# ZechengLi19/CIM

Hardware: AMD Instinct MI355X
Metric: images/sec training step (ResNet-50 VOC, ~1k proposals/img) at 1/2/4/8 GPU (higher is better)
Workload: dtype fp32

## Files before the change

### cim_amd/_lib.py

```python
import ctypes
import os

from ctypes import c_float, c_int, c_longlong, c_void_p

HERE = os.path.dirname(os.path.abspath(__file__))
LIB_PATH = os.environ.get("CIM_HIP_LIB") or os.path.join(HERE, "libcim_hip.so")

_P = c_void_p
SIGNATURES = {
    "cim_roi_align_fwd": [_P, _P, _P] + [c_int] * 6 + [c_float, c_int, c_int, _P],
    "cim_roi_align_fwd_ws": [_P, _P, _P] + [c_int] * 6 + [c_float, c_int, c_int, _P, _P],
    "cim_roi_align_maskcat_fwd_ws": [_P, _P, _P, _P] + [c_int] * 6 + [c_float, c_int, c_int, _P, _P],
    "cim_roi_align_wino7_pair_fwd": [_P, _P, _P, _P, _P] + [c_int] * 7 + [c_float, c_int, c_int, _P, _P],
    "cim_roi_align_bwd_ws": [_P, _P, _P] + [c_int] * 6 + [c_float, c_int, c_int, _P, c_int, _P, _P],
    "cim_roi_align_maskcat_bwd_ws": [_P, _P, _P, _P] + [c_int] * 6 + [c_float, c_int, c_int, _P, c_int, _P, _P],
    "cim_roi_align_bwd_workspace": [c_int, c_int, c_int, c_int],
    "cim_roi_align_bwd_scratch": [c_int, c_int, c_int, c_int, c_int],
    "cim_roi_align_bwd": [_P, _P, _P] + [c_int] * 6 + [c_float, c_int, c_int, _P, _P],
    "cim_roi_align_maskcat_fwd": [_P, _P, _P, _P] + [c_int] * 6 + [c_float, c_int, c_int, _P],
    "cim_roi_align_maskcat_bwd": [_P, _P, _P, _P] + [c_int] * 6 + [c_float, c_int, c_int, _P, _P],
    "cim_roi_align_forms": [c_int] * 9 + [_P] * 3,
    "cim_maxpool2d_out_size": [c_int, c_int, c_int, c_int],
    "cim_maxpool2d_fwd": [_P, _P, _P, c_int, c_int, c_int, c_int, c_int, c_int, _P],
    "cim_maxpool2d_bwd": [_P, _P, _P, c_int, c_int, c_int, c_int, c_int, c_int, _P],
    "cim_upsample_nearest_fwd": [_P, _P, c_int, c_int, c_int, c_int, c_int, _P],
    "cim_upsample_nearest_bwd": [_P, _P, c_int, c_int, c_int, c_int, _P],
    "cim_image_prep": [_P, c_int, c_int, _P, c_int, c_int, c_longlong, c_int, ctypes.c_double, c_int, _P, _P],
    "cim_mask_pack": [_P, _P, c_int, c_int, _P],
    "cim_mask_iou_pair": [_P, c_int, c_int, _P, _P, _P, _P],
    "cim_asy_flag": [_P, c_int, c_float, _P, _P],
    "cim_asy_prep": [_P, c_int, _P, c_int, _P, _P, _P],
    "cim_mining_step": [_P, _P, _P],
    "cim_mining_lds_bytes": [c_int, c_int],
    "cim_mining_sync_bytes": [],
    "cim_gemm_small_splits": [c_int, c_int, c_int],
    "cim_gemm_small_f32": [_P, _P, _P] + [c_int] * 8 + [_P, _P, _P, _P, _P, c_float, _P, c_int, c_int, _P, _P],
    "cim_conv1x1_bwd_workspace": [c_int, c_int, c_int, c_int],
    "cim_conv1x1_bn_act_bwd": [_P] * 8 + [c_float, c_int] + [_P] * 5 + [c_int] * 4 + [_P, _P, _P, _P, _P, c_int] + [c_int, _P, _P, c_float] + [_P] * 4 + [c_int],
    "cim_bn_part_finish": [_P, c_int, _P],
    "cim_conv3x3_nchw_splits": [c_int] * 5,
    "cim_conv3x3_nchw_f32": [_P, _P, _P] + [c_int] * 6 + [_P, _P, _P, _P, _P, c_float, _P, c_int, c_int, _P, _P],
    "cim_conv7x7_nchw_f32": [_P, _P, _P] + [c_int] * 5 + [_P, _P, _P, _P, c_float, c_int, _P],
    "cim_conv3x3_nchw_bwd_workspace": [c_int] * 6,
    "cim_conv3x3_dx_parts": [c_int] * 3,
    "cim_conv3x3_nchw_bn_act_bwd": [_P] * 8 + [c_float, c_int] + [_P] * 5 + [c_int] * 7 + [_P, _P, _P, _P, _P, c_int] + [c_int, _P, _P, c_float] + [_P] * 4,
    "cim_conv3x3_wt_multi": [_P, c_int, _P],
    "cim_bn_act_fwd": [_P, _P, _P, _P, _P, _P, c_float, _P, c_int, c_int, c_int, c_int, _P],
    "cim_bn_act_bwd_chunks": [c_int, c_int, c_int],
    "cim_bn_act_bwd": [_P, _P, _P, _P, _P, _P, c_float, _P, _P, _P, _P, c_int, c_int, c_int, c_int, _P],
    "cim_sgd_multi": [_P, _P, c_int, c_float, c_int, _P],
    "cim_adam_multi": [_P, _P, c_int, ctypes.c_double, ctypes.c_double, ctypes.c_double, c_int, _P],
    "cim_gemm_pair_splits": [c_int, c_int, c_int],
    "cim_gemm_pair": [_P, _P, _P, _P] + [c_int] * 6 + [c_int, c_int, c_int, c_int, _P, _P, _P, _P, c_int, c_int, c_int, _P],
    "cim_gemm_pair_batched": [_P, _P, _P] + [c_int] * 6 + [c_int, c_int, c_int, c_longlong, c_longlong, c_longlong,
                              _P, _P, c_int, c_int, c_int, _P],
    "cim_pair_scales": [_P, c_int, _P, _P, c_int, c_int, _P],
    "cim_pair_split": [_P, _P, c_int, c_int, c_int, c_int, c_int, c_int, c_longlong, c_longlong, _P, _P, _P],
    "cim_pair_amax": [_P, c_longlong, _P, _P],
    "cim_pair_masked_stats": [_P, _P, c_int, c_int, _P, _P, _P],
    "cim_wino7_flatten_bwd_dy_pair": [_P, _P, _P, _P, _P, _P, _P, c_int, c_int, c_int, _P],
    "cim_wino7_pair_scales": [_P, c_int, _P, c_int, _P, _P],
    "cim_wino7_input_pair": [_P, _P, _P, c_int, c_int, c_int, _P],
    "cim_wino7_filter_pair": [_P, _P, _P, c_int, c_int, _P],
    "cim_wino7_dy_pair": [_P, _P, _P, c_int, c_int, c_int, c_int, _P],
    "cim_wino7_output_amax": [_P, _P, _P, c_int, c_int, c_int, _P, _P],
    "cim_flatten_chw_pair": [_P, _P, _P, c_int, c_int, c_int, c_int, _P],
    "cim_flatten_chw_bwd_bias": [_P, _P, _P, _P, c_int, c_int, c_int, _P],
    "cim_wino_dx_adjoint_output": [_P, _P, c_int, c_int, c_int, c_int, _P],
    "cim_wino7_dx_maskfold": [_P, _P, _P, c_int, c_int, _P],
    "cim_wino_wgrad_output": [_P, _P, c_int, c_int, c_int, _P],
    "cim_losses_fwd": [_P, _P],
    "cim_linear_bias_f32": [_P, _P, _P, _P, c_int, c_int, c_int, c_int, _P, _P],
    "cim_loss_finish": [_P, c_int, _P, _P],
    "cim_loss_grad_combine": [_P] * 8 + [c_int, c_int, c_int, _P],
    "cim_head_act_fwd": [_P, _P, _P, c_int, c_int, c_int, _P],
    "cim_head_act_bwd": [_P, _P, _P, _P, c_int, c_int, c_int, _P],
    "cim_detect_ws_bytes": [c_int, c_int],
    "cim_detect_nms_limit": [_P, c_int, _P, c_int, c_int, c_float, c_float, c_int, _P, _P, _P, _P, _P],
    "cim_detect_corloc": [_P, c_int, c_int, c_int, _P, _P],
    "cim_batch_detect_ws_bytes": [_P, c_int, c_int],
    "cim_batch_detect_nms_limit": [_P, c_int, _P, _P, _P, c_int, c_int, c_float, c_float, c_int, _P, _P, _P, _P, _P, _P, _P],
    "cim_segm_words": [c_int, c_int],
    "cim_segm_pack": [_P, _P, c_longlong, c_int, c_int, c_int, _P, _P],
    "cim_segm_area": [_P, c_int, c_int, _P, _P],
    "cim_segm_rle_count": [_P, c_int, c_int, c_int, _P, _P],
    "cim_segm_rle_write": [_P, c_int, c_int, c_int, _P, _P, _P, _P],
    "cim_segm_rle_decode_ws_bytes": [c_longlong],
    "cim_segm_rle_decode": [_P, _P, _P, c_int, c_int, c_int, _P, _P, _P],
    "cim_segm_image_ws_bytes": [c_int, c_int, c_longlong],
    "cim_segm_record_bytes": [c_int, c_int, c_int, c_int],
    "cim_segm_eval_image": [_P, c_int, _P, c_int, c_int, _P, _P, c_int, c_int, c_int, c_longlong, _P, _P, _P, c_int, _P, c_int,
                            _P, _P, _P],
    "cim_segm_accumulate_ws_bytes": [c_longlong, c_int, c_int, c_int],
    "cim_segm_accumulate": [_P, c_int, c_longlong, c_int, _P, _P, _P, c_int, _P, c_int, _P, c_int, c_int, c_int, _P, _P, _P, _P,
                            _P],
# ... 80 lines not shown
```

### cim_amd/csrc/conv1x1.hip

```cpp
#include "common.h"
#include "../../include/cim_hip.h"

#ifndef CIM_BODY_PRIO_LEVEL
#define CIM_BODY_PRIO_LEVEL 3
#endif
#if CIM_BODY_PRIO_LEVEL > 0
#define CIM_BODY_PRIO() __builtin_amdgcn_s_setprio(CIM_BODY_PRIO_LEVEL)
#else
#define CIM_BODY_PRIO()
#endif
namespace {

#ifndef CIM_SMALL_BK
#define CIM_SMALL_BK 32
#endif
#ifndef CIM_SMALL_ABL
#define CIM_SMALL_ABL 0
#endif
constexpr int SBM = 64, SBN = 64, SBK = CIM_SMALL_BK;
constexpr int SLD = 68;
typedef float f32x16 __attribute__((ext_vector_type(16)));
typedef float f32x4u __attribute__((ext_vector_type(4), aligned(4)));
__device__ __forceinline__ float4 ld4(const float* p) {
    const f32x4u v = *reinterpret_cast<const f32x4u*>(p);
// ... 11 lines not shown
    const float* mask; const float* mgamma; const float* mvar; float meps;
    const float* mxr; const float* mmean; float* mpart; int mparts;
    int res_w, res_ws, res_hw;
};
struct InputBn { const float* y; const float* gamma; const float* var; float eps;
                 const float* xr; const float* mean; float* part; };

typedef unsigned int u32x4 __attribute__((ext_vector_type(4)));
typedef __amdgpu_buffer_rsrc_t rsrc_t;
__device__ __forceinline__ rsrc_t make_rsrc(const float* p, long long floats) {
    return __builtin_amdgcn_make_buffer_rsrc(const_cast<float*>(p), 0, (int)(unsigned)(floats * 4), 0x00020000);
}
__device__ __forceinline__ float4 bld4(rsrc_t r, unsigned byte_off) {
    const u32x4 v = __builtin_amdgcn_raw_buffer_load_b128(r, byte_off, 0, 0);
    return make_float4(__uint_as_float(v.x), __uint_as_float(v.y), __uint_as_float(v.z), __uint_as_float(v.w));
}
__device__ __forceinline__ float bld1(rsrc_t r, unsigned byte_off) {
    return __uint_as_float(__builtin_amdgcn_raw_buffer_load_b32(r, byte_off, 0, 0));
}
constexpr unsigned OOB = 0x7fffffffu;
__host__ __device__ __forceinline__ long long tile_extent(bool RC, int rows, int K, int ld) {
    return RC ? (long long)(K - 1) * ld + rows : (long long)(rows - 1) * ld + K;
}
template <bool RC, int ROWS>
__device__ __forceinline__ unsigned tile_off(int ld, int r0, int k0, int p) {
    int r, k;
    if (RC) { k = k0 + p / (ROWS / 4); r = r0 + (p % (ROWS / 4)) * 4; return ((unsigned)k * ld + r) * 4u; }
    r = r0 + p % ROWS; k = k0 + (p / ROWS) * 4;
    return ((unsigned)r * ld + k) * 4u;
}
template <bool RC, int ROWS>
__device__ __forceinline__ float4 tile_ktail(float4 v, int K, int k0, int p) {
    if (!RC) {
        const int left = K - (k0 + (p / ROWS) * 4);
        v.x = left > 0 ? v.x : 0.0f; v.y = left > 1 ? v.y : 0.0f; v.z = left > 2 ? v.z : 0.0f; v.w = left > 3 ? v.w : 0.0f;
    }
    return v;
}

template <bool RC, int ROWS>
__device__ __forceinline__ void tile_store(float* __restrict__ S, float4 v, int p) {
    if (RC) {
        const int k = p / (ROWS / 4), r = (p % (ROWS / 4)) * 4;
        *reinterpret_cast<float4*>(S + k * SLD + r) = v;
    } else {
        const int r = p % ROWS, k = (p / ROWS) * 4;
        S[(k + 0) * SLD + r] = v.x;
        S[(k + 1) * SLD + r] = v.y;
        S[(k + 2) * SLD + r] = v.z;
        S[(k + 3) * SLD + r] = v.w;
    }
}

__device__ __forceinline__ float small_value(const SmallArgs& g, int row, int col, float v, float& s1, float& s2) {
    const size_t o = (size_t)row * g.ldc + col;
    float y = v;
    if (g.bn) {
        const float a = g.gamma[row] * rsqrtf(g.var[row] + g.eps);
        y = fmaf(v, a, g.beta[row] - g.mean[row] * a);
    }
    if (g.res) {
        if (g.res_w == 0) y += g.res[o];
        else {
            const int py = col / g.res_w, px = col - py * g.res_w;
            if (!((py | px) & 1)) y += g.res[(size_t)row * g.res_hw + (py >> 1) * g.res_ws + (px >> 1)];
        }
    }
    if (g.colbias) y += g.colbias[col];
    if (g.relu) y = fmaxf(y, 0.0f);
    if (g.mask) {
        const bool on = g.mask[o] > 0.0f;
        if (g.mpart && on) { s1 += y; s2 = fmaf(y, g.mxr[o] - g.mmean[row], s2); }
        y = on ? y * (g.mgamma[row] * rsqrtf(g.mvar[row] + g.meps)) : 0.0f;
    }
    return y;
}
__device__ __forceinline__ void small_finish(const SmallArgs& g, int row, int col, float v, float& s1, float& s2) {
    const size_t o = (size_t)row * g.ldc + col;
    if (g.Xraw) g.Xraw[o] = v;
    g.C[o] = small_value(g, row, col, v, s1, s2);
}
__device__ __forceinline__ void small_finish(const SmallArgs& g, int row, int col, float v) {
    float s1 = 0.0f, s2 = 0.0f;
    small_finish(g, row, col, v, s1, s2);
}
__device__ __forceinline__ void small_put_part(const SmallArgs& g, int row, int group, int lane, float s1, float s2) {
#pragma unroll
    for (int o = 16; o > 0; o >>= 1) {
        s1 += __shfl_xor(s1, o);
        s2 += __shfl_xor(s2, o);
    }
    if ((lane & 31) == 0 && row < g.M && group < g.mparts) {
        g.mpart[(size_t)group * g.M + row] = s1;
        g.mpart[((size_t)g.mparts + group) * g.M + row] = s2;
    }
}
struct ColIdentity {
    static constexpr bool splitk = true;
    int N;
    __device__ __forceinline__ bool in(int c) const { return c < N; }
    __device__ __forceinline__ int col(int c) const { return c; }
    __device__ __forceinline__ int group(int c0) const { return c0 >> 5; }
};
struct ColParity {
    static constexpr bool splitk = false;
    int Wc, W, py, px, Nc, group0;
    __device__ __forceinline__ bool in(int c) const { return c < Nc; }
    __device__ __forceinline__ int col(int c) const {
        const int yc = c / Wc, xc = c - yc * Wc;
        return (2 * yc + py) * W + 2 * xc + px;
    }
    __device__ __forceinline__ int group(int c0) const { return group0 + (c0 >> 5); }
// ... 710 lines not shown
                   const float* residual, int relu, int splits, float* ws, hipStream_t st, int ksize = 3, const InputBn* in_bn = nullptr) {
    SmallArgs g = small_args(A, B, C, M, N, K, lda, 0, ldc, splits, ws, in_bn, x_raw, gamma, beta, mean, var, eps, residual, relu);
    g.b_kcontig = mode == CONV_DW;
    const dim3 grid((unsigned)(((M + SBM - 1) / SBM) * ((N + SBN - 1) / SBN)), (unsigned)splits);
    auto kern = ksize == 7 ? conv3x3_small_kernel<CONV_FWD, 7>
                : mode == CONV_FWD ? conv3x3_small_kernel<CONV_FWD> : mode == CONV_DX ? conv3x3_small_kernel<CONV_DX> : conv3x3_small_kernel<CONV_DW>;
    const int rc = launch_lds(kern, grid, sizeof(float) * 4 * CBK * SLD, st, g, c);
    if (rc) return rc;
    if (splits > 1) launch_splitk_reduce(g, st);
    return 0;
}
ConvGeom conv_geom(int cin, int cout, int H, int W, int stride, int mode, int dil = 1) {
    ConvGeom c;
    c.H = H; c.W = W; c.stride = stride; c.cin = cin; c.cout = cout; c.dil = dil;
    c.Ho = (H - 1) / stride + 1; c.Wo = (W - 1) / stride + 1;
    c.inv_w = 1.0f / (float)(mode == CONV_DX ? W : c.Wo);
    return c;
}
}

#define CONV3_ARGS_OK(CIN_MULT)                                                                                      \
    CIM_CHECK_ARG(cin > 0 && cout > 0 && H > 0 && W > 0 && (stride == 1 || stride == 2) && W <= 4096 &&               \
                  dilation >= 1 && dilation <= 8 && (dilation == 1 || stride == 1) &&                                 \
                  (long long)H * W < (1ll << 20) && (long long)cin * H * W < (1ll << 29) && (long long)cout * H * W < (1ll << 29) && \
                  (long long)cin * cout * 9 < (1ll << 29) && cin % (CIN_MULT) == 0)

extern "C" int cim_conv3x3_nchw_splits(int cin, int cout, int H, int W, int stride) {
    const int Ho = (H - 1) / stride + 1, Wo = (W - 1) / stride + 1;
    return cim_gemm_small_splits(cout, Ho * Wo, 9 * cin);
}

extern "C" int cim_conv3x3_nchw_f32(const float* x, const float* w, float* y, int cin, int cout, int H, int W, int stride,
                               int dilation, float* x_raw, const float* gamma, const float* beta, const float* mean, const float* var,
                               float eps, const float* residual, int relu, int splits, float* workspace, void* stream) {
    CIM_CHECK_ARG(x && w && y && splits >= 1 && splits <= 65535 && (splits == 1 || workspace));
    CONV3_ARGS_OK(1);
    CIM_CHECK_ARG((gamma == nullptr) == (beta == nullptr) && (gamma == nullptr) == (mean == nullptr) && (gamma == nullptr) == (var == nullptr));
    const ConvGeom c = conv_geom(cin, cout, H, W, stride, CONV_FWD, dilation);
    conv3x3_launch(CONV_FWD, w, x, y, cout, c.Ho * c.Wo, 9 * cin, 9 * cin, c.Ho * c.Wo, c, x_raw, gamma, beta, mean, var, eps,
                   residual, relu, splits, workspace, cim::as_stream(stream));
    CIM_CHECK_LAUNCH();
    return 0;
}

extern "C" int cim_conv7x7_nchw_f32(const float* x, const float* w, float* y, int cin, int cout, int H, int W, int stride,
                                    const float* gamma, const float* beta, const float* mean, const float* var, float eps,
                                    int relu, void* stream) {
    CIM_CHECK_ARG(x && w && y && cin > 0 && cout > 0 && H > 0 && W > 0 && (stride == 1 || stride == 2) && W <= 4096);
    CIM_CHECK_ARG((long long)H * W < (1ll << 20) && (long long)cin * H * W < (1ll << 29) && (long long)cout * H * W < (1ll << 29));
    CIM_CHECK_ARG((gamma == nullptr) == (beta == nullptr) && (gamma == nullptr) == (mean == nullptr) && (gamma == nullptr) == (var == nullptr));
    const ConvGeom c = conv_geom(cin, cout, H, W, stride, CONV_FWD);
    conv3x3_launch(CONV_FWD, w, x, y, cout, c.Ho * c.Wo, 49 * cin, 49 * cin, c.Ho * c.Wo, c, nullptr, gamma, beta, mean, var, eps,
                   nullptr, relu, 1, nullptr, cim::as_stream(stream), 7);
    CIM_CHECK_LAUNCH();
    return 0;
}

namespace {
Dx2Geom dx2_geom(int cin, int cout, int H, int W) {
    Dx2Geom c{};
    c.H = H; c.W = W; c.Ho = (H - 1) / 2 + 1; c.Wo = (W - 1) / 2 + 1; c.cin = cin; c.cout = cout;
    const int tiles_m = (cin + SBM - 1) / SBM;
    int first = 0, group = 0;
    for (int cls = 0; cls < 4; ++cls) {
        const int py = cls >> 1, px = cls & 1;
        const int nc = ((H - py + 1) / 2) * ((W - px + 1) / 2);
        c.first[cls] = first;
        c.tiles_n[cls] = (nc + SBN - 1) / SBN;
        c.group0[cls] = group;
        first += tiles_m * c.tiles_n[cls];
        group += 2 * c.tiles_n[cls];
    }
    c.first[4] = first;
    return c;
}
}

extern "C" int cim_conv3x3_dx_parts(int H, int W, int stride) {
    if (stride != 2) return (H * W + 31) / 32;
    int parts = 0;
    for (int cls = 0; cls < 4; ++cls) parts += 2 * ((((H - (cls >> 1) + 1) / 2) * ((W - (cls & 1) + 1) / 2) + SBN - 1) / SBN);
    return parts;
}

extern "C" long long cim_conv3x3_nchw_bwd_workspace(int B, int cin, int cout, int H, int W, int stride) {
    const int Ho = (H - 1) / stride + 1, Wo = (W - 1) / stride + 1;
    const long long dx = (long long)cim_gemm_small_splits(cin, H * W, 9 * cout) * cin * H * W;
    const long long dw = (long long)cim_gemm_small_splits(cout, 9 * cin, Ho * Wo) * cout * cin * 9 + (B > 1 ? (long long)cout * cin * 9 : 0);
    const long long dconv = (long long)B * cout * Ho * Wo;
    return (long long)sizeof(float) * (dconv + (long long)cout * cin * 9 + dx + dw);
}

extern "C" int cim_bn_part_finish(const cim_bn_part_desc* descs, int n, void* stream) {
    CIM_CHECK_ARG(descs && n > 0);
    hipStream_t st = cim::as_stream(stream);
    for (int base = 0; base < n; base += 24) {
        BnPartTable t{};
        t.n = n - base < 24 ? n - base : 24;
        int total = 0;
        for (int i = 0; i < t.n; ++i) {
            const cim_bn_part_desc& d = descs[base + i];
            CIM_CHECK_ARG(d.part && d.var && (d.dgamma || d.dbeta) && d.images > 0 && d.parts > 0 && d.channels > 0);
            t.d[i] = d;
            t.first[i] = total;
            total += (d.channels + 31) / 32;
        }
// ... 85 lines not shown
```

### cim_amd/modeling/resnet50.py

```python
import torch
import torch.nn as nn

from ..core.config import cfg
from ..ops import conv1x1_bn_act, conv3x3_bn_act, conv7x7_bn_act, max_pool2d
from ..ops.conv3x3 import prefetch_transposed_weights
from .maskfuse import MaskFuse


FUSE_BN_BWD = True


class Bottleneck(nn.Module):
    expansion = 4

    def __init__(self, inplanes, planes, stride=1, downsample=None):
        super().__init__()
        self.conv1 = nn.Conv2d(inplanes, planes, kernel_size=1, bias=False)
        self.bn1 = nn.BatchNorm2d(planes)
        self.conv2 = nn.Conv2d(planes, planes, kernel_size=3, stride=stride, padding=1, bias=False)
        self.bn2 = nn.BatchNorm2d(planes)
        self.conv3 = nn.Conv2d(planes, planes * 4, kernel_size=1, bias=False)
        self.bn3 = nn.BatchNorm2d(planes * 4)
        self.relu = nn.ReLU(inplace=True)
        self.downsample = downsample

    def forward(self, x):
        identity = x
        branch = {} if FUSE_BN_BWD else None
        out = conv1x1_bn_act(x, self.conv1, self.bn1, branch=branch)
        out = conv3x3_bn_act(out, self.conv2, self.bn2, fuse_input_bn=FUSE_BN_BWD)
        if self.downsample is not None:
            identity = conv1x1_bn_act(x, self.downsample[0], self.downsample[1], relu=False, branch=branch)
        return conv1x1_bn_act(out, self.conv3, self.bn3, residual=identity, fuse_input_bn=FUSE_BN_BWD, branch=branch)


def _make_layer(inplanes, planes, blocks, stride):
    downsample = None
    if stride != 1 or inplanes != planes * 4:
        downsample = nn.Sequential(nn.Conv2d(inplanes, planes * 4, kernel_size=1, stride=stride, bias=False),
                                   nn.BatchNorm2d(planes * 4))
    layers = [Bottleneck(inplanes, planes, stride, downsample)]
    for _ in range(1, blocks):
        layers.append(Bottleneck(planes * 4, planes))
    return nn.Sequential(*layers)


def freeze_params(m):
    for p in m.parameters():
        p.requires_grad = False


class resnet(nn.Module):
    def __init__(self, block_counts=4):
        super().__init__()
        if block_counts != 4:
            raise AssertionError
        self.res1 = nn.Sequential(nn.Conv2d(3, 64, kernel_size=7, stride=2, padding=3, bias=False),
                                  nn.BatchNorm2d(64), nn.ReLU(inplace=True),
                                  nn.MaxPool2d(kernel_size=3, stride=2, padding=1))
        self.res2 = _make_layer(64, 64, 3, 1)
        self.res3 = _make_layer(256, 128, 4, 2)
        self.res4 = _make_layer(512, 256, 6, 2)
        self.spatial_scale = 1 / 16
        self.dim_out = 1024
        self.block_counts = block_counts
        for m in self.modules():
            if isinstance(m, nn.Conv2d):
                nn.init.kaiming_normal_(m.weight, mode="fan_out", nonlinearity="relu")
        if cfg.MODEL.LOAD_IMAGENET_PRETRAINED_WEIGHTS:
            self.load_torchvision_state_dict(_torchvision_resnet50_state_dict())
            print("Load pre-trained weight for resnet !!")
        self._init_modules()

    def load_torchvision_state_dict(self, sd):
        ren = {"conv1.": "res1.0.", "bn1.": "res1.1.", "layer1.": "res2.", "layer2.": "res3.", "layer3.": "res4."}
        own = {}
        for k, v in sd.items():
            for a, b in ren.items():
                if k.startswith(a):
                    own[b + k[len(a):]] = v
        missing, unexpected = self.load_state_dict(own, strict=False)
        assert not unexpected and all("num_batches_tracked" in m for m in missing), (missing, unexpected)

    def _init_modules(self):
        assert cfg.ResNet.FREEZE_AT in [0, 2, 3, 4, 5]
        for i in range(1, cfg.ResNet.FREEZE_AT + 1):
            freeze_params(getattr(self, "res%d" % i))
        self.freeze(self)

    def freeze(self, m):
        for k in m.modules():
            if isinstance(k, nn.BatchNorm2d):
                k.eval()

    def train(self, mode=True):
        self.training = mode
        for i in range(cfg.ResNet.FREEZE_AT + 1, self.block_counts + 1):
            getattr(self, "res%d" % i).train(mode)
        self.freeze(self)
        return self

    def detectron_weight_mapping(self):
        return {name: name for name, _ in self.named_parameters()}, []

    def forward(self, x):
        if self.training and torch.is_grad_enabled():
            prefetch_transposed_weights([b.conv2 for i in range(cfg.ResNet.FREEZE_AT + 1, self.block_counts + 1)
                                         for b in getattr(self, "res%d" % i)])
        for i in range(self.block_counts):
            m = getattr(self, "res%d" % (i + 1))
            if i == 0:
                x = max_pool2d(conv7x7_bn_act(x, m[0], m[1], relu=True), m[3])
            else:
                x = m(x)
        return x


def _torchvision_resnet50_state_dict():
    try:
        from torchvision import models
    except ImportError as e:
        raise ImportError("cfg.MODEL.LOAD_IMAGENET_PRETRAINED_WEIGHTS for the ResNet body needs torchvision "
                          "(the reference wraps torchvision.models.resnet50, resnet50.py:12,20): %s" % e)
    return models.resnet50(pretrained=True).state_dict()


def torch_resnet50():
    return resnet()
```

### include/cim_hip.h

```cpp
#ifndef CIM_HIP_H
#define CIM_HIP_H

#include <stdint.h>

#ifdef __cplusplus
extern "C" {
#endif

const char* cim_last_error(void);
int cim_abi_version(void);

int cim_roi_align_fwd(const float* feat, const float* rois, float* out,
                      int B, int C, int H, int W, int K, int P,
                      float spatial_scale, int sampling_ratio, int aligned, void* stream);

long long cim_roi_align_bwd_workspace(int K, int P, int H, int W);
int cim_roi_align_bwd(const float* grad_out, const float* rois, float* grad_in,
                      int B, int C, int H, int W, int K, int P,
                      float spatial_scale, int sampling_ratio, int aligned, float* workspace, void* stream);

int cim_roi_align_fwd_ws(const float* feat, const float* rois, float* out,
                         int B, int C, int H, int W, int K, int P,
                         float spatial_scale, int sampling_ratio, int aligned, float* workspace, void* stream);
int cim_roi_align_maskcat_fwd_ws(const float* feat, const float* rois, const float* masks, float* cat,
// ... 123 lines not shown
#define CIM_VOC_MAX_RUN 256
long long cim_box_image_ws_bytes(int D, int G, long long pairs);
int cim_box_eval_image(const double* dt_box, int D, const double* gt_box, int G, const float* dt_score, const int32_t* meta,
                       int n_groups, int n_dl, int n_gl, long long pairs, const double* gt_area, const int64_t* gt_id,
                       const double* iou_thrs, int T, const double* area_rng, int A, void* ws, void* records, void* stream);
int cim_voc_match(const double* dt_box, const double* dt_conf, int D, const double* gt_box, const uint8_t* gt_difficult, int G,
                  const int32_t* groups, int n_groups, double ovthresh, int mode, uint8_t* tp, uint8_t* fp, double* ovmax,
                  int32_t* jmax, void* stream);
long long cim_voc_ap_ws_bytes(long long D);
int cim_voc_ap(const double* dt_conf, const uint8_t* tp, const uint8_t* fp, long long D, const int64_t* class_off,
               const double* npos, int K, const int64_t* runs, int n_runs, const int64_t* jobs, const int64_t* round_off,
               int rounds, const double* thr11, void* ws, double* rec, double* prec, double* ap, void* stream);

#define CIM_PROP_MAX_POINTS 256
#define CIM_PROP_MAX_S 16
long long cim_prop_ws_bytes(int N, int HW, int P);
int cim_prop_prepare(const uint8_t* masks_u8, int N, int H, int W, int S, uint64_t* packed, int32_t* boxes, int32_t* area,
                     uint8_t* small, int32_t* empty_flag, void* ws, void* stream);
int cim_prop_assign(const uint64_t* packed, const int32_t* area, int N, int H, int W, const int32_t* rows, const int32_t* cols,
                    const int32_t* classes, int P, int C, float* mat, void* ws, void* stream);

int cim_image_prep(const uint8_t* src_bgr, int h, int w, float* dst, int H, int W, long long plane_stride, int row_stride,
                   double inv_scale, int hflip, const float* mean_std6_host, void* stream);

int cim_maxpool2d_out_size(int in, int k, int stride, int pad);
int cim_maxpool2d_fwd(const float* x, float* y, int* idx, int NC, int H, int W, int k, int stride, int pad, void* stream);
int cim_maxpool2d_bwd(const float* dy, const int* idx, float* dx, int NC, int H, int W, int k, int stride, int pad, void* stream);
int cim_upsample_nearest_fwd(const float* x, float* y, int NC, int H, int W, int scale, int accumulate, void* stream);
int cim_upsample_nearest_bwd(const float* dy, float* dx, int NC, int H, int W, int scale, void* stream);

int cim_gemm_small_splits(int M, int N, int K);
int cim_gemm_small_f32(const float* A, const float* B, float* C, int M, int N, int K, int lda, int ldb, int ldc,
                       int a_mcontig, int b_kcontig, float* x_raw, const float* gamma, const float* beta,
                       const float* mean, const float* var, float eps, const float* residual, int relu, int splits,
                       float* workspace, void* stream);

long long cim_conv1x1_bwd_workspace(int B, int cin, int cout, int hw);
int cim_conv1x1_bn_act_bwd(const float* dy, const float* y, const float* x_raw, const float* x, const float* w,
                           const float* gamma, const float* mean, const float* var, float eps, int relu,
                           float* dres, float* dgamma, float* dbeta, float* dx, float* dw, int B, int cin, int cout, int hw,
                           float* workspace, void* stream, void* side_stream, void* fork_event, void* join_event, int join,
                           int dy_is_dconv, const float* in_gamma, const float* in_var, float in_eps,
                           const float* in_xr, const float* in_mean, float* in_part, const float* dx_add, int dx_add_w);
typedef struct { const float* part; const float* var; float eps; float* dgamma; float* dbeta; int images; int parts; int channels; } cim_bn_part_desc;
int cim_bn_part_finish(const cim_bn_part_desc* descs, int n, void* stream);

int cim_conv3x3_nchw_splits(int cin, int cout, int H, int W, int stride);
int cim_conv3x3_nchw_f32(const float* x, const float* w, float* y, int cin, int cout, int H, int W, int stride, int dilation,
                         float* x_raw, const float* gamma, const float* beta, const float* mean, const float* var, float eps,
                         const float* residual, int relu, int splits, float* workspace, void* stream);
int cim_conv7x7_nchw_f32(const float* x, const float* w, float* y, int cin, int cout, int H, int W, int stride,
                         const float* gamma, const float* beta, const float* mean, const float* var, float eps, int relu,
                         void* stream);
long long cim_conv3x3_nchw_bwd_workspace(int B, int cin, int cout, int H, int W, int stride);
int cim_conv3x3_dx_parts(int H, int W, int stride);
int cim_conv3x3_nchw_bn_act_bwd(const float* dy, const float* y, const float* x_raw, const float* x, const float* w,
                                const float* gamma, const float* mean, const float* var, float eps, int relu, float* dres,
                                float* dgamma, float* dbeta, float* dx, float* dw, int B, int cin, int cout, int H, int W,
                                int stride, int dilation, float* workspace, void* stream, void* side_stream, void* fork_event,
                                void* join_event, int join, int dy_is_dconv, const float* in_gamma, const float* in_var, float in_eps,
                                const float* in_xr, const float* in_mean, float* in_part, const float* wt_ready);
typedef struct { const float* w; float* wt; int cin; int cout; } cim_wt_desc;
int cim_conv3x3_wt_multi(const cim_wt_desc* descs, int n, void* stream);

int cim_bn_act_fwd(const float* x, const float* res, const float* gamma, const float* beta, const float* mean,
                   const float* var, float eps, float* y, int N, int C, int HW, int relu, void* stream);
int cim_bn_act_bwd_chunks(int N, int C, int HW);
int cim_bn_act_bwd(const float* dy, const float* y, const float* x, const float* gamma, const float* mean,
                   const float* var, float eps, float* dx, float* dres, float* dgamma, float* dbeta,
                   int N, int C, int HW, int relu, void* stream);

int cim_gemm_pair_splits(int M, int N, int K);
int cim_gemm_pair(const void* A, const void* B, float* C, const float* bias, int M, int N, int K,
                  int lda, int ldb, int ldc, int a_mcontig, int b_kcontig, int relu, int splits, float* workspace,
                  const float* a_scale, const float* b_scale, uint32_t* c_amax, int max_workgroups, int products, int form,
                  void* stream);
int cim_gemm_pair_batched(const void* A, const void* B, float* C, int M, int N, int K,
                          int lda, int ldb, int ldc, int a_mcontig, int b_kcontig,
                          int batch, long long a_bs, long long b_bs, long long c_bs,
                          const float* a_scale, const float* b_scale, int max_workgroups, int products, int form, void* stream);
int cim_pair_scales(const uint32_t* amax, int n_amax, const float* factor, float* scale, int n, int reduce_all, void* stream);
int cim_pair_split(const float* X, void* P, int rows, int rows_pad, int cols, int ld, int ldp, int batch,
                   long long x_bs, long long p_bs, const float* scale, const float* relu_y, void* stream);
int cim_pair_amax(const float* X, long long n, uint32_t* amax, void* stream);
int cim_pair_masked_stats(const float* dy, const float* y, int rows, int cols, float* part, uint32_t* amax, void* stream);

int cim_wino7_pair_scales(const uint32_t* amax, int n_amax, const uint32_t* amax_mul, int kind, float* scale, void* stream);
int cim_wino7_input_pair(const float* x, void* V, const float* scale, int R, int Rs, int C, void* stream);
int cim_wino7_filter_pair(const float* W, void* U, const float* scale, int Cout, int Cin, void* stream);
int cim_wino7_dy_pair(const float* dy, void* D, const float* scale, int R, int Rs, int C, int adjoint, void* stream);
int cim_wino7_flatten_bwd_dy_pair(const float* dX, const float* relu_y, void* E, const float* scale_e, void* D, const float* scale_d,
                                  float* bias_partial, int R, int Rs, int C, void* stream);
int cim_wino7_output_amax(const float* M, const float* bias, float* y, int R, int C, int relu, uint32_t* y_amax, void* stream);
int cim_flatten_chw_pair(const float* src, void* dst, const float* scale, int R, int Rs, int PP, int C, void* stream);
int cim_flatten_chw_bwd_bias(const float* src, const float* relu_y, float* dst, float* bias_partial, int R, int PP, int C,
                             void* stream);


int cim_wino_wgrad_output(const float* dU, float* dW, int Cout, int Cin, int tile, void* stream);
int cim_wino_dx_adjoint_output(const float* M, float* dx, int R, int P, int C, int tile, void* stream);
int cim_wino7_dx_maskfold(const float* M, const float* masks, float* dbox, int R, int Cb, void* stream);

#define CIM_PCL_MAX_CLUSTERS 256
typedef struct cim_loss_args {
    const float* pc;
    const float* pd;
// ... 63 lines not shown
```

Baseline: 76.86.

## Fuse frozen stem conv7x7+BN+ReLU+maxpool and frozen res2 bottleneck into single kernels

Adds a stem kernel that computes the 7x7 stride-2 conv, frozen BN, ReLU and 3x3 maxpool per output tile entirely in LDS. It also adds a fused bottleneck kernel that chains conv1x1, conv3x3 and conv1x1 with BN, ReLU, residual and optional downsample inside one block, using a halo tile. Both apply only when parameters are frozen and no input gradient is needed, as with ResNet stem/res2 in detection training. This removes the intermediate activation round trips to global memory and several launches, but adds per-image launches from Python and recomputes halo pixels for conv1.

Measured after the change: 77.13 (median of 2 runs). About the same (+0.4%).

```diff
diff --git a/cim_amd/_lib.py b/cim_amd/_lib.py
--- a/cim_amd/_lib.py
+++ b/cim_amd/_lib.py
@@ -41,6 +41,8 @@
     "cim_conv3x3_nchw_splits": [c_int] * 5,
     "cim_conv3x3_nchw_f32": [_P, _P, _P] + [c_int] * 6 + [_P, _P, _P, _P, _P, c_float, _P, c_int, c_int, _P, _P],
     "cim_conv7x7_nchw_f32": [_P, _P, _P] + [c_int] * 5 + [_P, _P, _P, _P, c_float, c_int, _P],
+    "cim_stem7x7_bn_relu_pool_f32": [_P, _P, _P] + [c_int] * 4 + [_P, _P, _P, _P, c_float, _P],
+    "cim_frozen_bottleneck_f32": [_P, _P, c_int, c_int, c_int, c_int, _P, _P, _P, _P, _P],
     "cim_conv3x3_nchw_bwd_workspace": [c_int] * 6,
     "cim_conv3x3_dx_parts": [c_int] * 3,
     "cim_conv3x3_nchw_bn_act_bwd": [_P] * 8 + [c_float, c_int] + [_P] * 5 + [c_int] * 7 + [_P, _P, _P, _P, _P, c_int] + [c_int, _P, _P, c_float] + [_P] * 4,
diff --git a/cim_amd/csrc/conv1x1.hip b/cim_amd/csrc/conv1x1.hip
--- a/cim_amd/csrc/conv1x1.hip
+++ b/cim_amd/csrc/conv1x1.hip
@@ -87,12 +87,21 @@
     }
 }
 
+__device__ __forceinline__ void bn_coeffs(const float* gamma, const float* beta, const float* mean, const float* var, float eps, int row,
+                                          float& a, float& b) {
+    a = gamma[row] * rsqrtf(var[row] + eps);
+    b = beta[row] - mean[row] * a;
+}
+__device__ __forceinline__ void small_bn_coeffs(const SmallArgs& g, int row, float& a, float& b) {
+    bn_coeffs(g.gamma, g.beta, g.mean, g.var, g.eps, row, a, b);
+}
 __device__ __forceinline__ float small_value(const SmallArgs& g, int row, int col, float v, float& s1, float& s2) {
     const size_t o = (size_t)row * g.ldc + col;
     float y = v;
     if (g.bn) {
-        const float a = g.gamma[row] * rsqrtf(g.var[row] + g.eps);
-        y = fmaf(v, a, g.beta[row] - g.mean[row] * a);
+        float a, b;
+        small_bn_coeffs(g, row, a, b);
+        y = fmaf(v, a, b);
     }
     if (g.res) {
         if (g.res_w == 0) y += g.res[o];
@@ -909,6 +918,356 @@
     const ConvGeom c = conv_geom(cin, cout, H, W, stride, CONV_FWD);
     conv3x3_launch(CONV_FWD, w, x, y, cout, c.Ho * c.Wo, 49 * cin, 49 * cin, c.Ho * c.Wo, c, nullptr, gamma, beta, mean, var, eps,
                    nullptr, relu, 1, nullptr, cim::as_stream(stream), 7);
+    CIM_CHECK_LAUNCH();
+    return 0;
+}
+
+namespace {
+constexpr int ST_CIN = 3, ST_K = 49 * ST_CIN, ST_KP = (ST_K + CBK - 1) / CBK * CBK;
+constexpr int ST_PH = 4, ST_PW = 8;
+constexpr int ST_CH = 2 * ST_PH + 1, ST_CW = 2 * ST_PW + 1, ST_NPIX = ST_CH * ST_CW;
+constexpr int ST_NT = (ST_NPIX + 31) / 32, ST_CLD = ST_NT * 32;
+constexpr int ST_XH = 2 * ST_CH + 5, ST_XW = 2 * ST_CW + 5, ST_XLD = ST_XW + 1;
+constexpr int ST_XZERO = ST_CIN * ST_XH * ST_XLD;
+static_assert(64 * ST_K <= 64 * ST_CLD, "the weights are staged in the convolution tile's LDS");
+struct StemGeom { int H, W, Hc, Wc, Hp, Wp, tiles_x; };
+__host__ __device__ constexpr int stem_koff(int k) {
+    return (k / 49) * ST_XH * ST_XLD + ((k % 49) / 7) * ST_XLD + (k % 49) % 7;
+}
+
+__global__ __launch_bounds__(256) void stem7x7_pool_kernel(const SmallArgs g, const StemGeom c) {
+    CIM_BODY_PRIO();
+    __shared__ __attribute__((aligned(16))) float cs[64 * ST_CLD];
+    __shared__ __attribute__((aligned(16))) float xs[ST_XZERO + 4];
+    __shared__ float ab[128];
+    const int tid = threadIdx.x, lane = tid & 63;
+    const int role = (tid >> 6) ^ (((int)blockIdx.x & 1) << 1);
+    const int wm = role & 1;
+    const int ph0 = ((int)blockIdx.x / c.tiles_x) * ST_PH, pw0 = ((int)blockIdx.x % c.tiles_x) * ST_PW;
+    const int cy0 = 2 * ph0 - 1, cx0 = 2 * pw0 - 1;
+    const int iy0 = 2 * cy0 - 3, ix0 = 2 * cx0 - 3;
+
+    for (int i = tid; i < g.M * ST_K; i += 256) cs[i] = g.A[i];
+    for (int i = tid; i < ST_CIN * ST_XH * ST_XW; i += 256) {
+        const int ch = i / (ST_XH * ST_XW), r = (i - ch * ST_XH * ST_XW) / ST_XW, cc = i - ch * ST_XH * ST_XW - r * ST_XW;
+        const int iy = iy0 + r, ix = ix0 + cc;
+        const bool ok = (unsigned)iy < (unsigned)c.H && (unsigned)ix < (unsigned)c.W;
+        xs[ch * ST_XH * ST_XLD + r * ST_XLD + cc] = ok ? g.B[(ch * c.H + iy) * c.W + ix] : 0.0f;
+    }
+    if (tid < 4) xs[ST_XZERO + tid] = 0.0f;
+    if (tid < 64) {
+        float a = 0.0f, b = 0.0f;
+        if (tid < g.M) small_bn_coeffs(g, tid, a, b);
+        ab[tid] = a;
+        ab[64 + tid] = b;
+    }
+    __syncthreads();
+    const int m = wm * 32 + (lane & 31), kk = lane >> 5;
+    float areg[ST_KP / 2];
+#pragma unroll
+    for (int t = 0; t < ST_KP / 2; ++t) {
+        const int k = 2 * t + kk;
+        const bool ok = m < g.M && k < ST_K;
+        const float v = cs[ok ? m * ST_K + k : 0];
+        areg[t] = ok ? v : 0.0f;
+    }
+    __syncthreads();
+
+    for (int nt = role >> 1; nt < ST_NT; nt += 2) {
+        const int n = nt * 32 + (lane & 31);
+        const int cyl = n / ST_CW, cxl = n - cyl * ST_CW;
+        const int pix = n < ST_NPIX ? 2 * cyl * ST_XLD + 2 * cxl : 0;
+        int odd = kk;
+        asm volatile("" : "+v"(odd));
+        f32x16 acc;
+#pragma unroll
+        for (int i = 0; i < 16; ++i) acc[i] = 0.0f;
+        constexpr int G = 8, NG = ST_KP / 2 / G;
+        float bv[2][G];
+        auto read_b = [&](int t0, float (&b)[G]) {
+#pragma unroll
+            for (int j = 0; j < G; ++j) {
+                const int t = t0 + j;
+                const int o0 = 2 * t < ST_K ? pix + stem_koff(2 * t) : ST_XZERO;
+                const int o1 = 2 * t + 1 < ST_K ? pix + stem_koff(2 * t + 1) : ST_XZERO;
+                b[j] = xs[odd ? o1 : o0];
+            }
+        };
+        read_b(0, bv[0]);
+#pragma unroll
+        for (int q = 0; q < NG; ++q) {
+            if (q + 1 < NG) read_b((q + 1) * G, bv[(q + 1) & 1]);
+#pragma unroll
+            for (int j = 0; j < G; ++j) acc = __builtin_amdgcn_mfma_f32_32x32x2f32(areg[q * G + j], bv[q & 1][j], acc, 0, 0, 0);
+            __builtin_amdgcn_sched_barrier(0);
+        }
+#pragma unroll
+        for (int r = 0; r < 16; ++r) {
+            const int row = wm * 32 + 8 * (r >> 2) + 4 * (lane >> 5) + (r & 3);
+            cs[row * ST_CLD + n] = fmaxf(fmaf(acc[r], ab[row], ab[64 + row]), 0.0f);
+        }
+    }
+    __syncthreads();
+
+    for (int i = tid; i < g.M * ST_PH * ST_PW; i += 256) {
+        const int pc = i % ST_PW, pr = (i / ST_PW) % ST_PH, ch = i / (ST_PH * ST_PW);
+        const int oh = ph0 + pr, ow = pw0 + pc;
+        if (oh >= c.Hp || ow >= c.Wp) continue;
+        const int h0 = max(oh * 2 - 1, 0), h1 = min(oh * 2 + 2, c.Hc);
+        const int w0 = max(ow * 2 - 1, 0), w1 = min(ow * 2 + 2, c.Wc);
+        float best = -INFINITY;
+        for (int h = h0; h < h1; ++h)
+            for (int w = w0; w < w1; ++w) {
+                const float v = cs[ch * ST_CLD + (h - cy0) * ST_CW + (w - cx0)];
+                if (v > best || v != v) best = v;
+            }
+        g.C[((size_t)ch * c.Hp + oh) * c.Wp + ow] = best;
+    }
+}
+}
+
+extern "C" int cim_stem7x7_bn_relu_pool_f32(const float* x, const float* w, float* y, int cin, int cout, int H, int W,
+                                            const float* gamma, const float* beta, const float* mean, const float* var, float eps,
+                                            void* stream) {
+    CIM_CHECK_ARG(x && w && y && gamma && beta && mean && var && cin == ST_CIN && cout > 0 && cout <= 64 && H > 0 && W > 0 && W <= 4096);
+    CIM_CHECK_ARG((long long)H * W < (1ll << 20));
+    StemGeom c;
+    c.H = H; c.W = W;
+    c.Hc = (H - 1) / 2 + 1; c.Wc = (W - 1) / 2 + 1;
+    c.Hp = (c.Hc - 1) / 2 + 1; c.Wp = (c.Wc - 1) / 2 + 1;
+    c.tiles_x = (c.Wp + ST_PW - 1) / ST_PW;
+    SmallArgs g = small_args(w, x, y, cout, c.Hc * c.Wc, ST_K, ST_K, 0, c.Hc * c.Wc, 1, nullptr, nullptr, nullptr, gamma, beta, mean, var, eps,
+                             nullptr, 1);
+    hipLaunchKernelGGL(stem7x7_pool_kernel, dim3((unsigned)(c.tiles_x * ((c.Hp + ST_PH - 1) / ST_PH))), dim3(256), 0,
+                       cim::as_stream(stream), g, c);
+    CIM_CHECK_LAUNCH();
+    return 0;
+}
+
+namespace {
+struct FbLayer { const float* w; const float* gamma; const float* beta; const float* mean; const float* var; float eps; };
+struct FbArgs { const float* x; float* y; FbLayer l1, l2, l3, ld; int cin, H, W, tiles_x, s1, s2; };
+constexpr int FB_T = 8, FB_HT = FB_T + 2, FB_NPX = FB_T * FB_T, FB_NH = 128, FB_P = 64;
+constexpr int FB_K2 = 9 * FB_P;
+constexpr size_t FB_LDS = sizeof(float) * (FB_P * FB_NH + FB_P * FB_NPX + 2 * 32 * SLD + FB_K2);
+
+template <class BF>
+__device__ __forceinline__ void fb_stream(rsrc_t RW, int ldw, int m0, int kbeg, int kend, float* __restrict__ As, int tid, int wm,
+                                          f32x16& acc, BF bf) {
+    const int lane = tid & 63, kk = lane >> 5, l31 = lane & 31;
+    const int nsl = (kend - kbeg) / 32, last = nsl - 1;
+    float4 ra[2];
+    unsigned oa[2];
+#pragma unroll
+    for (int i = 0; i < 2; ++i) oa[i] = tile_off<false, 64>(ldw, m0, kbeg, tid + i * 256);
+#pragma unroll
+    for (int i = 0; i < 2; ++i) ra[i] = bld4(RW, oa[i]);
+    __syncthreads();
+#pragma unroll
+    for (int i = 0; i < 2; ++i) tile_store<false, 64>(As, ra[i], tid + i * 256);
+#pragma unroll
+    for (int i = 0; i < 2; ++i) ra[i] = bld4(RW, oa[i] + (unsigned)min(1, last) * 128u);
+    __syncthreads();
+    for (int s = 0; s < nsl; ++s) {
+        const float* __restrict__ A = As + (s & 1) * 32 * SLD;
+        float av[16], bv[16];
+#pragma unroll
+        for (int t = 0; t < 16; ++t) {
+            av[t] = A[(2 * t + kk) * SLD + wm * 32 + l31];
+            bv[t] = bf(kbeg + s * 32 + 2 * t + kk);
+        }
+        if (s + 1 < nsl) {
+#pragma unroll
+            for (int i = 0; i < 2; ++i) tile_store<false, 64>(As + ((s + 1) & 1) * 32 * SLD, ra[i], tid + i * 256);
+        }
+#pragma unroll
+        for (int i = 0; i < 2; ++i) ra[i] = bld4(RW, oa[i] + (unsigned)min(s + 2, last) * 128u);
+#pragma unroll
+        for (int t = 0; t < 16; ++t) acc = __builtin_amdgcn_mfma_f32_32x32x2f32(av[t], bv[t], acc, 0, 0, 0);
+        __syncthreads();
+    }
+}
+__device__ __forceinline__ void fb_zero(f32x16& a) {
+#pragma unroll
+    for (int i = 0; i < 16; ++i) a[i] = 0.0f;
+}
+__device__ __forceinline__ void fb_add_split(f32x16& sum, const f32x16& acc, int seg) {
+#pragma unroll
+    for (int i = 0; i < 16; ++i) sum[i] = seg == 0 ? acc[i] : sum[i] + acc[i];
+}
+
+template <bool DS>
+__global__ __launch_bounds__(256, 2) void frozen_bottleneck_kernel(const FbArgs g) {
+    CIM_BODY_PRIO();
+    extern __shared__ __attribute__((aligned(16))) float fb_smem[];
+    float* a1s = fb_smem;
+    float* a2s = a1s + FB_P * FB_NH;
+    float* Bs = a2s;
+    float* xs = a1s;
+    float* As = a2s + FB_P * FB_NPX;
+    int* kofft = reinterpret_cast<int*>(As + 2 * 32 * SLD);
+    const int tid = threadIdx.x, lane = tid & 63, wave = tid >> 6, kk = lane >> 5, l31 = lane & 31;
+    const int H = g.H, W = g.W, HW = H * W, cin = g.cin;
+    const int ty0 = ((int)blockIdx.x / g.tiles_x) * FB_T, tx0 = ((int)blockIdx.x % g.tiles_x) * FB_T;
+    const rsrc_t RX = make_rsrc(g.x, (long long)cin * HW);
+
+    for (int k = tid; k < FB_K2; k += 256) {
+        const int ci = k / 9, tap = k - ci * 9;
+        kofft[k] = ci * FB_NH + (tap / 3) * FB_HT + tap % 3;
+    }
+
+    {
+        const rsrc_t RW = make_rsrc(g.l1.w, (long long)FB_P * cin);
+        const int ln = tid & 127, lk = tid >> 7;
+        const int liy = ty0 - 1 + ln / FB_HT, lix = tx0 - 1 + ln % FB_HT;
+        const bool lin = ln < FB_HT * FB_HT && (unsigned)liy < (unsigned)H && (unsigned)lix < (unsigned)W;
+        const unsigned lpix = (unsigned)(liy * W + lix);
+        const int kper = ((cin + g.s1 - 1) / g.s1 + 31) / 32 * 32;
+        f32x16 sum[2], acc[2];
+        for (int seg = 0; seg < g.s1; ++seg) {
+            const int kbeg = seg * kper, kend = min(cin, kbeg + kper);
+            const int nsl = (kend - kbeg) / 32;
+            fb_zero(acc[0]); fb_zero(acc[1]);
+            float4 ra[2];
+            float rb[16];
+            unsigned oa[2];
+#pragma unroll
+            for (int i = 0; i < 2; ++i) oa[i] = tile_off<false, 64>(cin, 0, kbeg, tid + i * 256);
+            auto gload = [&](int s) {
+#pragma unroll
+                for (int i = 0; i < 2; ++i) ra[i] = bld4(RW, oa[i] + (unsigned)s * 128u);
+#pragma unroll
+                for (int i = 0; i < 16; ++i)
+                    rb[i] = bld1(RX, lin ? ((unsigned)(kbeg + s * 32 + lk + 2 * i) * (unsigned)HW + lpix) * 4u : OOB);
+            };
+            gload(0);
+            for (int s = 0; s < nsl; ++s) {
+                __syncthreads();
+#pragma unroll
+                for (int i = 0; i < 2; ++i) tile_store<false, 64>(As, ra[i], tid + i * 256);
+#pragma unroll
+                for (int i = 0; i < 16; ++i) Bs[(lk + 2 * i) * FB_NH + ln] = rb[i];
+                __syncthreads();
+                gload(min(s + 1, nsl - 1));
+                float av0[16], av1[16], bv[16];
+#pragma unroll
+                for (int t = 0; t < 16; ++t) {
+                    av0[t] = As[(2 * t + kk) * SLD + l31];
+                    av1[t] = As[(2 * t + kk) * SLD + 32 + l31];
+                    bv[t] = Bs[(2 * t + kk) * FB_NH + wave * 32 + l31];
+                }
+#pragma unroll
+                for (int t = 0; t < 16; ++t) {
+                    acc[0] = __builtin_amdgcn_mfma_f32_32x32x2f32(av0[t], bv[t], acc[0], 0, 0, 0);
+                    acc[1] = __builtin_amdgcn_mfma_f32_32x32x2f32(av1[t], bv[t], acc[1], 0, 0, 0);
+                }
+            }
+            fb_add_split(sum[0], acc[0], seg);
+            fb_add_split(sum[1], acc[1], seg);
+        }
+        const int n = wave * 32 + l31;
+        const int iy = ty0 - 1 + n / FB_HT, ix = tx0 - 1 + n % FB_HT;
+        const bool in = n < FB_HT * FB_HT && (unsigned)iy < (unsigned)H && (unsigned)ix < (unsigned)W;
+#pragma unroll
+        for (int mt = 0; mt < 2; ++mt)
+#pragma unroll
+            for (int r = 0; r < 16; ++r) {
+                const int row = mt * 32 + 8 * (r >> 2) + 4 * kk + (r & 3);
+                float a, b;
+                bn_coeffs(g.l1.gamma, g.l1.beta, g.l1.mean, g.l1.var, g.l1.eps, row, a, b);
+                a1s[row * FB_NH + n] = in ? fmaxf(fmaf(sum[mt][r], a, b), 0.0f) : 0.0f;
+            }
+    }
+
+    const int wm = wave >> 1, wn = wave & 1;
+    const int n = wn * 32 + l31, py = n >> 3, px = n & 7;
+    const int oy = ty0 + py, ox = tx0 + px;
+    const bool pin = oy < H && ox < W;
+    {
+        const rsrc_t RW = make_rsrc(g.l2.w, (long long)FB_P * FB_K2);
+        const int base = py * FB_HT + px;
+        const int kper = ((FB_K2 + g.s2 - 1) / g.s2 + 31) / 32 * 32;
+        f32x16 sum, acc;
+        for (int seg = 0; seg < g.s2; ++seg) {
+            const int kbeg = seg * kper, kend = min(FB_K2, kbeg + kper);
+            fb_zero(acc);
+            fb_stream(RW, FB_K2, 0, kbeg, kend, As, tid, wm, acc, [&](int k) { return a1s[kofft[k] + base]; });
+            fb_add_split(sum, acc, seg);
+        }
+#pragma unroll
+        for (int r = 0; r < 16; ++r) {
+            const int row = wm * 32 + 8 * (r >> 2) + 4 * kk + (r & 3);
+            float a, b;
+            bn_coeffs(g.l2.gamma, g.l2.beta, g.l2.mean, g.l2.var, g.l2.eps, row, a, b);
+            a2s[row * FB_NPX + n] = fmaxf(fmaf(sum[r], a, b), 0.0f);
+        }
+    }
+
+    if (DS) {
+        const int tn = tid & 63, tk = tid >> 6;
+        const int yy = ty0 + (tn >> 3), xx = tx0 + (tn & 7);
+        const bool ok = yy < H && xx < W;
+        float rb[16];
+#pragma unroll
+        for (int i = 0; i < 16; ++i) rb[i] = bld1(RX, ok ? ((unsigned)(tk + 4 * i) * (unsigned)HW + (unsigned)(yy * W + xx)) * 4u : OOB);
+        __syncthreads();
+#pragma unroll
+        for (int i = 0; i < 16; ++i) xs[(tk + 4 * i) * FB_NPX + tn] = rb[i];
+    }
+    const rsrc_t RW3 = make_rsrc(g.l3.w, (long long)4 * FB_P * FB_P);
+    const rsrc_t RWD = make_rsrc(DS ? g.ld.w : g.l3.w, (long long)4 * FB_P * FB_P);
+    for (int mc = 0; mc < 4; ++mc) {
+        f32x16 idv, acc;
+        if (DS) {
+            fb_zero(acc);
+            fb_stream(RWD, FB_P, mc * 64, 0, FB_P, As, tid, wm, acc, [&](int k) { return xs[k * FB_NPX + n]; });
+#pragma unroll
+            for (int r = 0; r < 16; ++r) {
+                const int row = mc * 64 + wm * 32 + 8 * (r >> 2) + 4 * kk + (r & 3);
+                float a, b;
+                bn_coeffs(g.ld.gamma, g.ld.beta, g.ld.mean, g.ld.var, g.ld.eps, row, a, b);
+                idv[r] = fmaf(acc[r], a, b);
+            }
+        }
+        fb_zero(acc);
+        fb_stream(RW3, FB_P, mc * 64, 0, FB_P, As, tid, wm, acc, [&](int k) { return a2s[k * FB_NPX + n]; });
+        if (pin) {
+#pragma unroll
+            for (int r = 0; r < 16; ++r) {
+                const int row = mc * 64 + wm * 32 + 8 * (r >> 2) + 4 * kk + (r & 3);
+                const size_t o = (size_t)row * HW + oy * W + ox;
+                float a, b;
+                bn_coeffs(g.l3.gamma, g.l3.beta, g.l3.mean, g.l3.var, g.l3.eps, row, a, b);
+                float y = fmaf(acc[r], a, b);
+                y += DS ? idv[r] : g.x[o];
+                g.y[o] = fmaxf(y, 0.0f);
+            }
+        }
+    }
+}
+}
+
+extern "C" int cim_frozen_bottleneck_f32(const float* x, float* y, int cin, int planes, int H, int W, const cim_conv_bn* conv1,
+                                         const cim_conv_bn* conv2, const cim_conv_bn* conv3, const cim_conv_bn* downsample, void* stream) {
+    CIM_CHECK_ARG(x && y && conv1 && conv2 && conv3 && planes == FB_P && H > 0 && W > 0 && W <= 4096 && (long long)H * W < (1ll << 20));
+    CIM_CHECK_ARG(downsample ? cin == FB_P : cin == 4 * FB_P);
+    const cim_conv_bn* ls[4] = {conv1, conv2, conv3, downsample};
+    FbArgs g{};
+    FbLayer* out[4] = {&g.l1, &g.l2, &g.l3, &g.ld};
+    for (int i = 0; i < 4; ++i) {
+        if (!ls[i]) continue;
+        CIM_CHECK_ARG(ls[i]->w && ls[i]->gamma && ls[i]->beta && ls[i]->mean && ls[i]->var);
+        *out[i] = FbLayer{ls[i]->w, ls[i]->gamma, ls[i]->beta, ls[i]->mean, ls[i]->var, ls[i]->eps};
+    }
+    g.x = x; g.y = y; g.cin = cin; g.H = H; g.W = W;
+    g.tiles_x = (W + FB_T - 1) / FB_T;
+    g.s1 = cim_gemm_small_splits(FB_P, H * W, cin);
+    g.s2 = cim_gemm_small_splits(FB_P, H * W, FB_K2);
+    CIM_CHECK_ARG(cim_gemm_small_splits(4 * FB_P, H * W, FB_P) == 1 && g.s1 <= 2 && g.s2 <= 4);
+    const dim3 grid((unsigned)(g.tiles_x * ((H + FB_T - 1) / FB_T)));
+    const int rc = downsample ? launch_lds(frozen_bottleneck_kernel<true>, grid, FB_LDS, cim::as_stream(stream), g)
+                              : launch_lds(frozen_bottleneck_kernel<false>, grid, FB_LDS, cim::as_stream(stream), g);
+    if (rc) { cim::set_error("%s: hipFuncSetAttribute failed (%d)", __func__, rc); return rc; }
     CIM_CHECK_LAUNCH();
     return 0;
 }
diff --git a/cim_amd/modeling/resnet50.py b/cim_amd/modeling/resnet50.py
--- a/cim_amd/modeling/resnet50.py
+++ b/cim_amd/modeling/resnet50.py
@@ -4,10 +4,13 @@
 from ..core.config import cfg
 from ..ops import conv1x1_bn_act, conv3x3_bn_act, conv7x7_bn_act, max_pool2d
 from ..ops.conv3x3 import prefetch_transposed_weights
+from ..ops.frozen import bottleneck as frozen_bottleneck, stem_bn_relu_pool
 from .maskfuse import MaskFuse
 
 
 FUSE_BN_BWD = True
+FUSE_FROZEN = True
+FUSE_FROZEN_BLOCKS = True
 
 
 class Bottleneck(nn.Module):
@@ -25,6 +28,10 @@
         self.downsample = downsample
 
     def forward(self, x):
+        if FUSE_FROZEN_BLOCKS:
+            y = frozen_bottleneck(x, self)
+            if y is not None:
+                return y
         identity = x
         branch = {} if FUSE_BN_BWD else None
         out = conv1x1_bn_act(x, self.conv1, self.bn1, branch=branch)
@@ -110,7 +117,8 @@
         for i in range(self.block_counts):
             m = getattr(self, "res%d" % (i + 1))
             if i == 0:
-                x = max_pool2d(conv7x7_bn_act(x, m[0], m[1], relu=True), m[3])
+                y = stem_bn_relu_pool(x, m[0], m[1], m[3]) if FUSE_FROZEN else None
+                x = y if y is not None else max_pool2d(conv7x7_bn_act(x, m[0], m[1], relu=True), m[3])
             else:
                 x = m(x)
         return x
diff --git a/cim_amd/ops/frozen.py b/cim_amd/ops/frozen.py
--- /dev/null
+++ b/cim_amd/ops/frozen.py
@@ -0,0 +1,92 @@
+import ctypes
+
+import torch
+
+from .. import _lib
+
+
+def eligible(bn_eval, param_requires_grad, input_requires_grad, grad_enabled, stride, planes, dense_fp32_gpu):
+    return bool(bn_eval and not param_requires_grad and not (input_requires_grad and grad_enabled)
+                and stride == 1 and planes <= 64 and dense_fp32_gpu)
+
+
+def facts(x, convs, bns, stride, planes):
+    params = [p for m in list(convs) + list(bns) for p in m.parameters()]
+    tensors = [x] + params + [b for m in bns for b in (m.running_mean, m.running_var) if b is not None]
+    return dict(bn_eval=all((not m.training) and m.affine and m.track_running_stats for m in bns),
+                param_requires_grad=any(p.requires_grad for p in params),
+                input_requires_grad=x.requires_grad, grad_enabled=torch.is_grad_enabled(),
+                stride=stride, planes=planes,
+                dense_fp32_gpu=all(t.is_cuda and t.dtype == torch.float32 and t.is_contiguous() for t in tensors))
+
+
+def _pair(v):
+    return (v, v) if isinstance(v, int) else tuple(v)
+
+
+def stem_bn_relu_pool(x, conv, bn, pool):
+    geometry = (x.dim() == 4 and conv.in_channels == 3 and conv.kernel_size == (7, 7) and conv.stride == (2, 2)
+                and conv.padding == (3, 3) and conv.dilation == (1, 1) and conv.groups == 1 and conv.bias is None
+                and _pair(pool.kernel_size) == (3, 3) and _pair(pool.stride) == (2, 2) and _pair(pool.padding) == (1, 1)
+                and _pair(pool.dilation) == (1, 1) and not pool.ceil_mode and not pool.return_indices
+                and x.shape[3] <= 4096 and x.shape[2] * x.shape[3] < (1 << 20))
+    if not (geometry and eligible(**facts(x, [conv], [bn], 1, conv.out_channels))):
+        return None
+    with torch.no_grad():
+        B, cin, H, W = x.shape
+        cout = conv.out_channels
+        hc, wc = (H - 1) // 2 + 1, (W - 1) // 2 + 1
+        y = torch.empty((B, cout, (hc - 1) // 2 + 1, (wc - 1) // 2 + 1), dtype=torch.float32, device=x.device)
+        for b in range(B):
+            _lib.call("cim_stem7x7_bn_relu_pool_f32", x[b].data_ptr(), conv.weight.data_ptr(), y[b].data_ptr(), cin, cout, H, W,
+                      bn.weight.data_ptr(), bn.bias.data_ptr(), bn.running_mean.data_ptr(), bn.running_var.data_ptr(),
+                      float(bn.eps), _lib.stream_ptr())
+    return y
+
+
+class _ConvBn(ctypes.Structure):
+    _fields_ = [("w", ctypes.c_void_p), ("gamma", ctypes.c_void_p), ("beta", ctypes.c_void_p), ("mean", ctypes.c_void_p),
+                ("var", ctypes.c_void_p), ("eps", ctypes.c_float)]
+
+
+def _conv_bn(conv, bn):
+    return _ConvBn(conv.weight.data_ptr(), bn.weight.data_ptr(), bn.bias.data_ptr(), bn.running_mean.data_ptr(),
+                   bn.running_var.data_ptr(), float(bn.eps))
+
+
+def _plain(conv, k, stride):
+    return (conv.kernel_size == (k, k) and conv.stride == (stride, stride) and conv.padding == (k // 2, k // 2)
+            and conv.dilation == (1, 1) and conv.groups == 1 and conv.bias is None)
+
+
+DISPATCH_IDENTITY_FORM = False
+
+
+def bottleneck(x, block, identity_form=None):
+    if block.downsample is None and not (DISPATCH_IDENTITY_FORM if identity_form is None else identity_form):
+        return None
+    planes, stride = block.conv2.out_channels, block.conv2.stride[0]
+    if planes != 64 or stride != 1 or block.conv1.weight.requires_grad:
+        return None
+    convs, bns = [block.conv1, block.conv2, block.conv3], [block.bn1, block.bn2, block.bn3]
+    ds = block.downsample
+    if ds is not None:
+        convs, bns = convs + [ds[0]], bns + [ds[1]]
+    cin = block.conv1.in_channels
+    geometry = (x.dim() == 4 and planes == 64 and block.conv1.out_channels == 64 and block.conv2.in_channels == 64
+                and block.conv3.in_channels == 64 and block.conv3.out_channels == 256 and x.shape[1] == cin
+                and _plain(block.conv1, 1, 1) and _plain(block.conv2, 3, stride) and _plain(block.conv3, 1, 1)
+                and ((ds is None and cin == 256) or (ds is not None and cin == 64 and len(ds) == 2 and _plain(ds[0], 1, 1)
+                                                     and ds[0].in_channels == 64 and ds[0].out_channels == 256))
+                and x.shape[3] <= 4096 and x.shape[2] * x.shape[3] < (1 << 20))
+    if not (geometry and eligible(**facts(x, convs, bns, stride, planes))):
+        return None
+    with torch.no_grad():
+        B, _, H, W = x.shape
+        y = torch.empty((B, 256, H, W), dtype=torch.float32, device=x.device)
+        descs = [_conv_bn(c, b) for c, b in zip(convs, bns)]
+        for b in range(B):
+            _lib.call("cim_frozen_bottleneck_f32", x[b].data_ptr(), y[b].data_ptr(), cin, planes, H, W, ctypes.byref(descs[0]),
+                      ctypes.byref(descs[1]), ctypes.byref(descs[2]), ctypes.byref(descs[3]) if ds is not None else None,
+                      _lib.stream_ptr())
+    return y
diff --git a/include/cim_hip.h b/include/cim_hip.h
--- a/include/cim_hip.h
+++ b/include/cim_hip.h
@@ -199,6 +199,12 @@
 int cim_conv7x7_nchw_f32(const float* x, const float* w, float* y, int cin, int cout, int H, int W, int stride,
                          const float* gamma, const float* beta, const float* mean, const float* var, float eps, int relu,
                          void* stream);
+int cim_stem7x7_bn_relu_pool_f32(const float* x, const float* w, float* y, int cin, int cout, int H, int W,
+                                 const float* gamma, const float* beta, const float* mean, const float* var, float eps,
+                                 void* stream);
+typedef struct { const float* w; const float* gamma; const float* beta; const float* mean; const float* var; float eps; } cim_conv_bn;
+int cim_frozen_bottleneck_f32(const float* x, float* y, int cin, int planes, int H, int W, const cim_conv_bn* conv1,
+                              const cim_conv_bn* conv2, const cim_conv_bn* conv3, const cim_conv_bn* downsample, void* stream);
 long long cim_conv3x3_nchw_bwd_workspace(int B, int cin, int cout, int H, int W, int stride);
 int cim_conv3x3_dx_parts(int H, int W, int stride);
 int cim_conv3x3_nchw_bn_act_bwd(const float* dy, const float* y, const float* x_raw, const float* x, const float* w,
```
